# daveredrum/D3Net

Measured on AMD Instinct MI355X. Metric: scenes/sec fwd+bwd (PointGroup+speaker), higher is better.
Workload: dtype bf16

## Files before the change

d3net_amd/_lib.py:

```python
import ctypes as C
import os

_HERE = os.path.dirname(os.path.abspath(__file__))
SO_PATH = os.path.join(_HERE, "lib", "libd3hip.so")

ERRORS = {-1: "D3_ERR_WORKSPACE", -2: "D3_ERR_RANGE (coordinate/batch outside key range)",
          -3: "D3_ERR_ARG", -4: "D3_ERR_OVERFLOW"}


class D3Error(RuntimeError):
    pass


_lib = None
vp, i32, i64, f32, sz = C.c_void_p, C.c_int, C.c_longlong, C.c_float, C.c_size_t
f64 = C.c_double
pi = C.POINTER(C.c_int)

SIGNATURES = {
    "d3_version": (i32, []),
    "d3_arch": (C.c_char_p, []),
    "d3_sec_mean": (i32, [vp, vp, vp, i32, i32, vp]),
    "d3_sec_min": (i32, [vp, vp, vp, i32, i32, vp]),
    "d3_sec_max": (i32, [vp, vp, vp, i32, i32, vp]),
# ... 84 lines not shown
    "d3_point_heads_ws_bytes": (sz, []),
    "d3_point_heads_fwd": (i32, [vp, i64, i32, i32, vp, vp, vp, vp, vp, vp, vp, vp, f32, f32, i32, vp, vp, vp, vp, vp, vp, vp, vp, vp,
                                 vp, sz, vp]),
    "d3_score_loss": (i32, [vp, vp, i32, i32, f32, f32, vp, vp, vp, vp]),
    "d3_query_locals_mask": (i32, [vp, vp, i32, i32, i32, vp]),
    "d3_caption_select_target": (i32, [vp, vp, vp, i32, i32, i32, i32, vp, vp, vp, vp]),
    "d3_caption_inputs_fwd": (i32, [vp, vp, vp, vp, vp, i32, i32, i32, i32, i32, vp, vp, vp, vp, vp]),
    "d3_caption_inputs_bwd": (i32, [vp, vp, vp, vp, i32, i32, i32, i32, i32, vp, vp, vp]),
    "d3_masked_xe_ws_bytes": (sz, [i32, i32]),
    "d3_masked_xe": (i32, [vp, vp, i64, vp, i32, i32, i32, vp, vp, vp, sz, vp]),
    "d3_orientation_loss": (i32, [vp, i64, i64, vp, vp, vp, vp, vp, vp, i32, i32, i32, i32, i32, vp, i32, vp, vp, vp]),
    "d3_offset_loss_ws_bytes": (sz, []),
    "d3_offset_loss": (i32, [vp, vp, vp, i32, vp, i64, vp, vp, vp, i32, vp, sz, vp]),
    "d3_scatter_add_rows": (i32, [vp, vp, vp, i64, i32, vp]),
    "d3_gather_rows": (i32, [vp, vp, vp, i64, i32, vp]),
    "d3_cross_entropy_ws_bytes": (sz, []),
    "d3_cross_entropy": (i32, [vp, vp, vp, vp, i32, i32, i32, vp, sz, vp]),
    "d3_attn_fwd": (i32, [vp, vp, vp, vp, vp, vp, vp, i32, i32, i32, i32, i32, i32, i32, vp]),
    "d3_attn_bwd": (i32, [vp, vp, vp, vp, vp, vp, vp, vp, vp, i32, i32, i32, i32, i32, i32, vp]),
    "d3_hgemm": (i32, [vp, i32, vp]),
    "d3_colsum_ws_bytes": (sz, [i32]),
    "d3_colsum": (i32, [vp, i64, i32, i32, vp, i32, vp, sz, vp]),
    "d3_topdown_ws_bytes": (sz, [i32, i32, i32, i32, i32, i32]),
    "d3_topdown_bwd_ws_bytes": (sz, [i32, i32, i32, i32, i32, i32, i32]),
    "d3_topdown_xe_forward": (i32, [vp, vp]),
    "d3_topdown_xe_backward": (i32, [vp, vp, vp]),
    "d3_topdown_xe_backward_ex": (i32, [vp, vp, vp, vp]),
    "d3_topdown_step_ws_bytes": (sz, [i32, i32, i32, i32, i32]),
    "d3_topdown_feat_proj": (i32, [vp, vp, vp, i32, i32, i32, vp]),
    "d3_topdown_step": (i32, [vp, vp, vp, i32, vp, vp, vp, vp, vp, vp, vp, sz, vp]),
    "d3_beam_select": (i32, [vp, vp, i32, i32, i32, i32, i32, i32, i32, i32, vp, vp, vp, vp, vp, vp, vp, vp, vp, vp, i32, vp]),
    "d3_greedy_select": (i32, [vp, i32, i32, vp, vp, vp]),
    "d3_topdown_greedy": (i32, [vp, vp, i32, vp, vp, vp, vp, vp, vp, vp, sz, vp, i32, vp, vp, vp]),
    "d3_topdown_beam": (i32, [vp, vp, i32, vp, vp, vp, vp, vp, sz, vp, i32, i32, vp, vp, vp, vp, vp, vp, vp]),
    "d3_topdown_beam_greedy": (i32, [vp, vp, i32, vp, vp, vp, vp, vp, sz, vp, i32, i32, vp, vp, vp, vp, vp, vp, i32, vp, vp, vp]),
    "d3_gru_seq_ws_bytes": (sz, [i32, i32, i32, i32]),
    "d3_gru_seq_bwd_ws_bytes": (sz, [i32, i32, i32, i32]),
    "d3_gru_seq_forward": (i32, [vp, vp, vp, vp, vp, vp, i32, i32, i32, i32, vp, vp, vp, sz, vp]),
    "d3_gru_seq_backward": (i32, [vp, vp, vp, vp, i32, i32, i32, i32, vp, vp, vp, vp, vp, vp, vp, vp, vp, sz, vp]),
    "d3_nms3d_samecls": (i32, [vp, vp, vp, i32, i32, f64, i32, vp, vp]),
    "d3_instance_cross_iou": (i32, [vp, vp, i64, i32, i32, vp, vp, vp, vp]),
    "d3_nms_matrix": (i32, [vp, vp, vp, i32, f32, vp, vp, vp, vp]),
    "d3_seg_eval_max_inst": (i32, []),
    "d3_seg_eval_ws_bytes": (sz, [i32, i32]),
    "d3_seg_eval": (i32, [vp, vp, vp, vp, i32, i32, i32, i32, vp, i32, vp, vp, i32, i64, C.c_ulonglong, vp, vp, vp, vp, vp, vp, sz, vp]),
    "d3_scene_limits": (i32, [pi, pi, pi]),
# ... 124 lines not shown
```

d3net_amd/csrc/topdown.hip:

```cpp
#include "common.h"
#include "prof.h"
#include <string.h>

typedef float f32x4 __attribute__((ext_vector_type(4)));
#ifndef GRU_U
#define GRU_U 2
#endif

int hg_launch(const d3_gemm_prob *probs, int nprobs, hipStream_t s);
size_t hg_colsum_ws_bytes(int njobs, int cmax);
int hg_colsum_multi(const float *const *x, const long long *ld, const int *R, const int *C, float *const *out, const int *accum, int n,
                    void *ws, size_t ws_bytes, hipStream_t s);

struct GruArgs {
    const float *x; long long ldx; int I;
    const float *h; long long ldh;
    const float *Wih, *Whh, *bih, *bhh;
    float *hout; long long ldo;
    float *r, *z, *n, *ghn;
    int N, H;
    const float *gi_pre; long long ldgi;
    const int *lens; int t_step;
    float *hid_out; long long ldhid;
    const float *xb; long long ldxb; int Ib; long long ldw;
// ... 235 lines not shown
                                        float *__restrict__ dgi, long long lddgi, float *__restrict__ dgh, float *__restrict__ dhp,
                                        int N, int H, const int *__restrict__ lens, int t_step) {
    const int e = blockIdx.x * blockDim.x + threadIdx.x;
    if (e >= N * H) return;
    const int row = e / H, c = e - row * H;
    float dh = 0.f;
    if (d0) dh += d0[(long long)row * ld0 + c];
    if (d1 && !(lens && t_step >= lens[row])) dh += d1[(long long)row * ld1 + c];
    if (d2) dh += d2[(long long)row * ld2 + c];
    const float rr = r[e], zz = z[e], nv = n[e];
    const float dn = dh * (1.f - zz), dz = dh * (hp[(long long)row * ldh + c] - nv);
    const float dnp = dn * (1.f - nv * nv);
    const float drp = dnp * ghn[e] * rr * (1.f - rr);
    const float dzp = dz * zz * (1.f - zz);
    const long long o = (long long)row * 3 * H + c, oi = (long long)row * lddgi + c;
    dgi[oi] = drp; dgi[oi + H] = dzp; dgi[oi + 2 * H] = dnp;
    dgh[o] = drp; dgh[o + H] = dzp; dgh[o + 2 * H] = dnp * rr;
    dhp[e] = dh * zz;
}

#define TD_PREP_T 1024
__global__ __launch_bounds__(TD_PREP_T) void td_attn_prep_kernel(const float *__restrict__ mask, const float *__restrict__ obj,
                                                                 int *__restrict__ act, int *__restrict__ nact, float *__restrict__ msum,
                                                                 int K, int F, int obj_div) {
    extern __shared__ float sm[];
    const int n = blockIdx.x, t = threadIdx.x, lane = t & 63;
    const long long ns = n / obj_div;
    if (t < 64) {
        int base = 0;
        for (int k0 = 0; k0 < K; k0 += 64) {
            const int k = k0 + lane;
            const bool on = k < K && mask[(long long)n * K + k] != 0.f;
            const unsigned long long bal = __ballot(on);
            if (on) act[(long long)n * K + base + __popcll(bal & ((1ull << lane) - 1ull))] = k;
            base += __popcll(bal);
        }
        if (lane == 0) nact[n] = base;
    }
    const int nsl = TD_PREP_T / F, sl = t / F, c = t - sl * F;
    if (sl < nsl) {
        const int per = (K + nsl - 1) / nsl, k0 = sl * per, k1 = min(K, k0 + per);
        float s = 0.f;
        int k = k0;
        for (; k + 4 <= k1; k += 4) {
            float v[4], m[4];
#pragma unroll
            for (int q = 0; q < 4; q++) { v[q] = obj[(ns * K + k + q) * F + c]; m[q] = mask[(long long)n * K + k + q]; }
#pragma unroll
            for (int q = 0; q < 4; q++) s += (m[q] == 0.f) ? v[q] : 0.f;
        }
        for (; k < k1; k++)
            if (mask[(long long)n * K + k] == 0.f) s += obj[(ns * K + k) * F + c];
        sm[sl * F + c] = s;
    }
    __syncthreads();
    if (t < F) {
        float s = sm[t];
        for (int q = 1; q < nsl; q++) s += sm[q * F + t];
        msum[(long long)n * F + t] = s;
    }
}

#ifndef TD_ATT_T
#define TD_ATT_T 1024
#endif
static inline size_t td_attn_bwd_rsum_floats(int H) { const int CT = H < TD_ATT_T ? H : TD_ATT_T, RS = TD_ATT_T / CT; return RS > 1 ? (size_t)RS * 2 * H : 0; }
template <int NTH>
__global__ __launch_bounds__(NTH) void td_attn_fwd_kernel(const float *__restrict__ fp, const float *__restrict__ q, long long ldq,
                                                          const float *__restrict__ watt, const float *__restrict__ obj,
                                                          const int *__restrict__ act, const int *__restrict__ nact,
                                                          const float *__restrict__ msum, float *__restrict__ a_out,
                                                          float *__restrict__ att, long long ldatt, float *__restrict__ attn_out,
                                                          int t_step, int S, int K, int H, int F, int obj_div) {
    extern __shared__ float sm[];
    float *qs = sm, *ws = qs + H, *sc = ws + H, *ak = sc + K, *part = ak + K;
    __shared__ float am_s;
    const int n = blockIdx.x, t = threadIdx.x, lane = t & 63, wave = t >> 6;
    const long long ns = n / obj_div;
    const int na = nact[n], nm = K - na;
    const int *al = act + (long long)n * K;
    for (int c = t; c < H; c += NTH) { qs[c] = q[(long long)n * ldq + c]; ws[c] = watt[c]; }
    __syncthreads();
    for (int j = wave; j < na; j += NTH / 64) {
        const float *row = fp + (ns * K + al[j]) * H;
        float s = 0.f;
        for (int c = lane * 4; c < H; c += 256) {
            const f32x4 v = *(const f32x4 *)(row + c);
#pragma unroll
            for (int u = 0; u < 4; u++) s += ws[c + u] * tanhf(v[u] + qs[c + u]);
        }
        for (int o = 32; o > 0; o >>= 1) s += __shfl_xor(s, o);
        if (lane == 0) sc[j] = s;
    }
    __syncthreads();
    if (wave == 0) {
        float mx = nm > 0 ? 0.f : -3.0e38f;
        for (int j = lane; j < na; j += 64) mx = fmaxf(mx, sc[j]);
        for (int o = 32; o > 0; o >>= 1) mx = fmaxf(mx, __shfl_xor(mx, o));
        float sum = 0.f;
        for (int j = lane; j < na; j += 64) { const float e = expf(sc[j] - mx); sc[j] = e; sum += e; }
        for (int o = 32; o > 0; o >>= 1) sum += __shfl_xor(sum, o);
        const float e0 = expf(-mx);
        sum += (float)nm * e0;
        const float inv = 1.f / sum;
        for (int j = lane; j < na; j += 64) sc[j] *= inv;
        if (lane == 0) am_s = e0 * inv;
    }
    __syncthreads();
    const float am = am_s;
    for (int k = t; k < K; k += NTH) ak[k] = am;
    __syncthreads();
    for (int j = t; j < na; j += NTH) ak[al[j]] = sc[j];
    __syncthreads();
    for (int k = t; k < K; k += NTH) {
        a_out[(long long)n * K + k] = ak[k];
        if (attn_out) attn_out[((long long)n * K + k) * S + t_step] = ak[k];
    }
    const int half = t / F, c = t - half * F;
    if (half < 2) {
        const int j0 = half * ((na + 1) / 2), j1 = min(na, j0 + (na + 1) / 2);
        float s = 0.f;
        for (int j = j0; j < j1; j++) s += sc[j] * obj[(ns * K + al[j]) * F + c];
        part[half * F + c] = s;
    }
    __syncthreads();
    if (t < F) att[(long long)n * ldatt + t] = am * msum[(long long)n * F + t] + (part[t] + part[F + t]);
}

template <int NTH>
__global__ __launch_bounds__(NTH) void td_attn_bwd_kernel(const float *__restrict__ datt, long long lddatt, const float *__restrict__ a_in,
                                                          const float *__restrict__ att, long long ldatt, const float *__restrict__ fp,
                                                          const float *__restrict__ q, long long ldq, const float *__restrict__ watt,
                                                          const float *__restrict__ obj, const int *__restrict__ act,
                                                          const int *__restrict__ nact, float *__restrict__ dq, long long lddq,
                                                          float *__restrict__ dfp, float *__restrict__ dwpart, float *__restrict__ dattS,
                                                          int K, int H, int F) {
    extern __shared__ float sm[];
    float *dat = sm, *dss = dat + F, *red = dss + K, *rsum = red + 4;
    const int n = blockIdx.x, t = threadIdx.x, lane = t & 63, wave = t >> 6;
    const int na = nact[n];
    const int *al = act + (long long)n * K;
    float pd = 0.f;
    for (int c = t; c < F; c += NTH) {
        const float v = datt[(long long)n * lddatt + c];
        dat[c] = v; dattS[(long long)n * F + c] = v;
        pd += v * att[(long long)n * ldatt + c];
    }
    for (int o = 32; o > 0; o >>= 1) pd += __shfl_xor(pd, o);
    if (lane == 0 && wave < 4) red[wave] = pd;
    __syncthreads();
    const float dot = (red[0] + red[1]) + (red[2] + red[3]);
    for (int j = wave; j < na; j += NTH / 64) {
        const int k = al[j];
        float s = 0.f;
        for (int c = lane; c < F; c += 64) s += dat[c] * obj[((long long)n * K + k) * F + c];
        for (int o = 32; o > 0; o >>= 1) s += __shfl_xor(s, o);
        if (lane == 0) dss[j] = a_in[(long long)n * K + k] * (s - dot);
    }
    __syncthreads();
    const int CT = H < NTH ? H : NTH, RS = NTH / CT, rs = t / CT;
    for (int c = t - rs * CT; c < H && rs < RS; c += CT) {
        const float qc = q[(long long)n * ldq + c], wc = watt[c];
        float dqa = 0.f, dwa = 0.f;
        for (int j0 = rs * 4; j0 < na; j0 += 4 * RS) {
            float fv[4], dv[4];
            long long o[4];
#pragma unroll
            for (int u = 0; u < 4; u++) {
                const int j = j0 + u < na ? j0 + u : j0;
                o[u] = ((long long)n * K + al[j]) * H + c;
                fv[u] = fp[o[u]]; dv[u] = dfp[o[u]];
            }
#pragma unroll
            for (int u = 0; u < 4; u++) {
                if (j0 + u < na) {
                    const float ds = dss[j0 + u];
                    const float th = tanhf(fv[u] + qc);
                    const float dp = ds * wc * (1.f - th * th);
                    dfp[o[u]] = dv[u] + dp;
                    dqa += dp; dwa += ds * th;
                }
            }
        }
        if (rs == 0 && RS == 1) { dq[(long long)n * lddq + c] = dqa; dwpart[(long long)n * H + c] = dwa; }
        else if (rs > 0) { rsum[((rs - 1) * 2) * H + c] = dqa; rsum[((rs - 1) * 2 + 1) * H + c] = dwa; }
        else { rsum[(RS - 1) * 2 * H + c] = dqa; rsum[(RS - 1) * 2 * H + H + c] = dwa; }
    }
    if (RS > 1) {
        __syncthreads();
        for (int c = t; c < H; c += NTH) {
            float dqa = rsum[(RS - 1) * 2 * H + c], dwa = rsum[(RS - 1) * 2 * H + H + c];
            for (int r = 1; r < RS; r++) { dqa += rsum[((r - 1) * 2) * H + c]; dwa += rsum[((r - 1) * 2 + 1) * H + c]; }
            dq[(long long)n * lddq + c] = dqa;
            dwpart[(long long)n * H + c] = dwa;
        }
    }
}

__global__ __launch_bounds__(256) void td_dobj_kernel(const float *__restrict__ a, const float *__restrict__ dattS, float *__restrict__ dobj,
                                                      int S, int N, int K, int F, int SC) {
    extern __shared__ float sm[];
    float *aS = sm, *dS = aS + (size_t)SC * K;
    const int n = blockIdx.x, t = threadIdx.x;
    const int c = t % F, kb = t / F, kst = 256 / F;
    for (int s0 = 0; s0 < S; s0 += SC) {
        const int sc = min(SC, S - s0);
        __syncthreads();
        for (int e = t; e < sc * K; e += 256) { const int tt = e / K, k = e - tt * K; aS[e] = a[((long long)(s0 + tt) * N + n) * K + k]; }
        for (int e = t; e < sc * F; e += 256) { const int tt = e / F, cc = e - tt * F; dS[e] = dattS[((long long)(s0 + tt) * N + n) * F + cc]; }
        __syncthreads();
        const int kper = (K + gridDim.y - 1) / gridDim.y, k0 = blockIdx.y * kper, k1 = min(K, k0 + kper);
        for (int k = k0 + kb; k < k1; k += kst) {
            float v = 0.f;
            for (int tt = 0; tt < sc; tt++) v += aS[tt * K + k] * dS[tt * F + c];
            float *o = dobj + ((long long)n * K + k) * F + c;
            *o = s0 == 0 ? v : *o + v;
        }
    }
// ... 20 lines not shown
    const long long e = (long long)blockIdx.x * blockDim.x + threadIdx.x;
    if (e < n && c0[e] <= 0.f) d[e] = 0.f;
}
__global__ void td_sum_time_kernel(const float *__restrict__ x, float *__restrict__ out, int S, int N, int C) {
    const int e = blockIdx.x * blockDim.x + threadIdx.x;
    if (e >= N * C) return;
    float s = 0.f;
    for (int tt = 0; tt < S; tt++) s += x[(long long)tt * N * C + e];
    out[e] = s;
}

static d3_gemm_seg td_seg(const float *A, long long lda, const float *B, long long ldb, int K, const int *ia = nullptr, int akm = 0, int bkm = 0) {
    d3_gemm_seg s;
    s.A = A; s.ia = ia; s.lda = lda; s.a_kmajor = akm; s.B = B; s.ldb = ldb; s.b_kmajor = bkm; s.K = K;
    return s;
}
static d3_gemm_prob td_prob(int M, int N, float *C, long long ldc) {
    d3_gemm_prob p;
    memset(&p, 0, sizeof(p));
    p.M = M; p.N = N; p.C = C; p.ldc = ldc;
    return p;
}

struct TdLayout {
    size_t widx, nidx, bidx, act, nact, msum, fp, TD, x1, x2, H1, H2, g1, g2, q, a, att, c0, gi1, Wa, Wb, bc2, total;
};
static TdLayout td_layout(int N, int K, int S, int H, int E, int F) {
    TdLayout L;
    size_t o = 0;
    const size_t R = (size_t)S * N;
    auto take = [&](size_t bytes) { size_t at = o; o += d3_align(bytes); return at; };
    L.widx = take(R * 4); L.nidx = take(R * 4); L.bidx = take(R * 4);
    L.act = take((size_t)N * K * 4); L.nact = take((size_t)N * 4); L.msum = take((size_t)N * F * 4);
    L.fp = take((size_t)N * K * H * 4);
    L.TD = take(R * E * 4); L.x1 = take(R * E * 4); L.x2 = take(R * E * 4);
    L.H1 = take((R + N) * H * 4); L.H2 = take((R + N) * H * 4);
    L.g1 = take(4 * R * H * 4); L.g2 = take(4 * R * H * 4);
    L.q = take(R * H * 4); L.a = take(R * K * 4); L.att = take(R * F * 4); L.c0 = take(R * H * 4);
    L.gi1 = take(R * 3 * H * 4); L.Wa = take((size_t)3 * H * (F + H) * 4); L.Wb = take((size_t)3 * H * H * 4); L.bc2 = take((size_t)3 * H * 4);
    L.total = o;
    return L;
}

extern "C" size_t d3_topdown_ws_bytes(int N, int K, int S, int H, int E, int F) {
    return td_layout(N, K, S, H, E, F).total;
}

static int td_check(const d3_topdown_args *a) {
    if (!a || a->N < 1 || a->K < 1 || a->S < 1 || a->V < 1 || a->S > a->Tw) return D3_ERR_ARG;
    if ((a->H & 15) || (a->E & 3) || (a->F & 3) || a->F > 128 || (256 % a->F) || a->K > 1024) return D3_ERR_ARG;
    if (a->ws_bytes < td_layout(a->N, a->K, a->S, a->H, a->E, a->F).total) return D3_ERR_WORKSPACE;
    return 0;
}

extern "C" int d3_topdown_xe_forward(const d3_topdown_args *a, void *stream) {
    D3_CLEAR();
    int rc = td_check(a);
    if (rc) return rc;
    hipStream_t s = d3_stream(stream);
    const int N = a->N, K = a->K, S = a->S, V = a->V, H = a->H, E = a->E, F = a->F, R = S * N;
    const TdLayout L = td_layout(N, K, S, H, E, F);
    char *ws = (char *)a->ws;
    int *widx = (int *)(ws + L.widx), *nidx = (int *)(ws + L.nidx), *bidx = (int *)(ws + L.bidx);
    float *fp = (float *)(ws + L.fp), *TD = (float *)(ws + L.TD), *x1 = (float *)(ws + L.x1), *x2 = (float *)(ws + L.x2);
    float *H1 = (float *)(ws + L.H1), *H2 = (float *)(ws + L.H2), *g1 = (float *)(ws + L.g1), *g2 = (float *)(ws + L.g2);
    float *q = (float *)(ws + L.q), *av = (float *)(ws + L.a), *att = (float *)(ws + L.att), *c0 = (float *)(ws + L.c0);
    int *act = (int *)(ws + L.act), *nact = (int *)(ws + L.nact);
    float *msum = (float *)(ws + L.msum);
    const long long ldtd = H + F + E;
    const long long ldlang = F + H;
    td_rows_kernel<<<(R + 255) / 256, 256, 0, s>>>(a->word_ids, a->Tw, N, S, V, widx, nidx, bidx);
    td_attn_prep_kernel<<<N, TD_PREP_T, (size_t)(TD_PREP_T / F) * F * 4, s>>>(a->mask, a->obj, act, nact, msum, K, F, 1);
    D3_CHECK(hipMemsetAsync(H1, 0, (size_t)N * H * 4, s));
    D3_CHECK(hipMemsetAsync(H2, 0, (size_t)N * H * 4, s));
    {
        d3_gemm_prob p[2];
        p[0] = td_prob(N * K, H, fp, H);
        p[0].nseg = 1; p[0].seg[0] = td_seg(a->obj, F, a->W_feat, F, F);
        p[1] = td_prob(R, E, TD, E);
        p[1].nseg = 2;
        p[1].seg[0] = td_seg(a->emb, E, a->W_td, ldtd, E, widx);
        p[1].seg[1] = td_seg(a->target, F, a->W_td + E + H, ldtd, F, nidx);
        p[1].bias = a->b_td;
        if ((rc = hg_launch(&p[0], 1, s))) return rc;
        if ((rc = hg_launch(&p[1], 1, s))) return rc;
    }
    float *gi1 = (float *)(ws + L.gi1), *Wa = (float *)(ws + L.Wa), *Wb = (float *)(ws + L.Wb), *bc2 = (float *)(ws + L.bc2);
    {
        d3_gemm_prob p[4];
        p[0] = td_prob(3 * H, F + H, Wa, F + H);
        p[0].nseg = 1; p[0].seg[0] = td_seg(a->Wih2, E, a->W_lang, ldlang, E, nullptr, 0, 1);
        p[1] = td_prob(3 * H, H, Wb, H);
        p[1].nseg = 1; p[1].seg[0] = td_seg(a->Wih1, E, a->W_td + E, ldtd, E, nullptr, 0, 1);
        p[2] = td_prob(3 * H, 1, bc2, 1);
        p[2].nseg = 1; p[2].seg[0] = td_seg(a->Wih2, E, a->b_lang, E, E);
        p[2].add = a->bih2; p[2].ldadd = 1;
        p[3] = td_prob(R, 3 * H, gi1, 3 * H);
        p[3].nseg = 1; p[3].seg[0] = td_seg(TD, E, a->Wih1, E, E);
        p[3].bias = a->bih1;
        if ((rc = hg_launch(p, 3, s))) return rc;
        if ((rc = hg_launch(&p[3], 1, s))) return rc;
    }
    const size_t RH = (size_t)R * H;
    for (int t = 0; t < S; t++) {
        const size_t rN = (size_t)t * N;
        float *h1p = H1 + rN * H, *h1n = H1 + (rN + N) * H, *h2p = H2 + rN * H, *h2n = H2 + (rN + N) * H;
        {
            GruArgs g{h2p, H, H, h1p, H, Wb, a->Whh1, nullptr, a->bhh1, h1n, H,
                      g1 + rN * H, g1 + RH + rN * H, g1 + 2 * RH + rN * H, g1 + 3 * RH + rN * H, N, H, gi1 + rN * 3 * H, 3 * H, nullptr, 0, nullptr, 0,
                      nullptr, 0, 0, H};
            if ((rc = td_gru_fwd(g, s))) return rc;
        }
        {
            d3_gemm_prob p = td_prob(N, H, q + rN * H, H);
            p.nseg = 1; p.seg[0] = td_seg(h1n, H, a->W_hidd, H, H);
            if ((rc = hg_launch(&p, 1, s))) return rc;
        }
        td_attn_fwd_kernel<TD_ATT_T><<<N, TD_ATT_T, (size_t)(2 * H + 2 * K + 2 * F) * 4, s>>>(fp, q + rN * H, H, a->w_att, a->obj, act, nact, msum, av + rN * K,
                                                                             att + rN * F, F, a->attn, t, S, K, H, F, 1);
        {
            GruArgs g{att + rN * F, F, F, h2p, H, Wa, a->Whh2, bc2, a->bhh2, h2n, H,
                      g2 + rN * H, g2 + RH + rN * H, g2 + 2 * RH + rN * H, g2 + 3 * RH + rN * H, N, H, nullptr, 0, nullptr, 0, nullptr, 0,
                      h1n, H, H, F + H};
            if ((rc = td_gru_fwd(g, s))) return rc;
        }
    }
    {
        d3_gemm_prob p[2];
        p[0] = td_prob(R, E, x1, E);
        p[0].nseg = 1; p[0].seg[0] = td_seg(H2, H, a->W_td + E, ldtd, H);
        p[0].add = TD; p[0].ldadd = E;
        p[1] = td_prob(R, E, x2, E);
        p[1].nseg = 2;
        p[1].seg[0] = td_seg(att, F, a->W_lang, ldlang, F);
        p[1].seg[1] = td_seg(H1 + (size_t)N * H, H, a->W_lang + F, ldlang, H);
        p[1].bias = a->b_lang;
        if ((rc = hg_launch(p, 2, s))) return rc;
    }
    {
        d3_gemm_prob p = td_prob(R, H, c0, H);
        p.nseg = 1; p.seg[0] = td_seg(H2 + (size_t)N * H, H, a->Wc0, H, H);
        p.bias = a->bc0; p.relu = 1;
// ... 75 lines not shown
    if ((rc = fork(0))) return rc;
    {
        const long long tot = (long long)R * V;
        td_gather_rows_kernel<<<(int)((tot + 255) / 256), 256, 0, sp>>>(gd->dlogits, bidx, dlog, R, V);
        d3_gemm_prob p[3];
        p[0] = td_prob(V, H, gd->dWc2, H);
        p[0].nseg = 1; p[0].seg[0] = td_seg(dlog, V, c0, H, R, nullptr, 1, 1);
        p[1] = td_prob(H, H, gd->dWc0, H);
        p[1].nseg = 1; p[1].seg[0] = td_seg(dc0, H, H2 + (size_t)N * H, H, R, nullptr, 1, 1);
        p[2] = td_prob(R, H, dH2, H);
        p[2].nseg = 1; p[2].seg[0] = td_seg(dc0, H, a->Wc0, H, H, nullptr, 0, 1);
        if ((rc = hg_launch(&p[2], 1, s))) return rc;
        if ((rc = hg_launch(&p[0], 1, sp))) return rc;
        if ((rc = hg_launch(&p[1], 1, sp))) return rc;
        const float *cx[2] = {dlog, dc0}; const long long cl[2] = {V, H}; const int cr[2] = {R, R}, cc[2] = {V, H};
        float *co[2] = {gd->dbc2, gd->dbc0};
        if ((rc = hg_colsum_multi(cx, cl, cr, cc, co, nullptr, 2, bw + B.cs, B.cs_bytes, sp))) return rc;
    }
    D3_CHECK(hipMemsetAsync(dh1c, 0, (size_t)N * H * 4, s));
    D3_CHECK(hipMemsetAsync(dh2c, 0, (size_t)N * H * 4, s));
    D3_CHECK(hipMemsetAsync(dfp, 0, (size_t)N * K * H * 4, s));
    const int nh = (N * H + 255) / 256;
    const bool fuse = d3_tune(D3T_TD_FUSE_GATES) != 0;
    auto gates_epi = [&](d3_gemm_prob &p, const float *d0, long long ld0, const float *d1, long long ld1, const float *g, size_t rN,
                         const float *hp, float *dgi, float *dgh, float *dhp) {
        p.gru = 1; p.gru_H = H;
        p.g_d0 = d0; p.g_ld0 = ld0; p.g_d1 = d1; p.g_ld1 = ld1;
        p.g_r = g + rN * H; p.g_z = g + RH + rN * H; p.g_n = g + 2 * RH + rN * H; p.g_ghn = g + 3 * RH + rN * H;
        p.g_hp = hp; p.g_ldh = H;
        p.g_dgi = dgi; p.g_lddgi = 3 * H; p.g_dgh = dgh; p.g_dhp = dhp;
    };
    for (int t = S - 1; t >= 0; t--) {
        const size_t rN = (size_t)t * N;
        float *h1p = H1 + rN * H, *h2p = H2 + rN * H;
        if (!fuse || t == S - 1)
            td_gru_bwd_gates_kernel<<<nh, 256, 0, s>>>(dH2 + rN * H, H, dh2c, H, nullptr, 0, g2 + rN * H, g2 + RH + rN * H, g2 + 2 * RH + rN * H,
                                                       g2 + 3 * RH + rN * H, h2p, H, dgi2 + rN * 3 * H, 3 * H, dgh2 + rN * 3 * H, dh2c, N, H, nullptr, 0);
        {
            d3_gemm_prob p[3];
            p[0] = td_prob(N, H, dh2c, H);
            p[0].nseg = 1; p[0].seg[0] = td_seg(dgh2 + rN * 3 * H, 3 * H, a->Whh2, H, 3 * H, nullptr, 0, 1); p[0].accum = 1;
            p[1] = td_prob(N, F + H, tmpL, F + H);
            p[1].nseg = 1; p[1].seg[0] = td_seg(dgi2 + rN * 3 * H, 3 * H, Wa, F + H, 3 * H, nullptr, 0, 1);
            p[2] = td_prob(N, E, dx2 + rN * E, E);
            p[2].nseg = 1; p[2].seg[0] = td_seg(dgi2 + rN * 3 * H, 3 * H, a->Wih2, E, 3 * H, nullptr, 0, 1);
            if ((rc = hg_launch(p, 3, s))) return rc;
        }
        td_attn_bwd_kernel<TD_ATT_T><<<N, TD_ATT_T, (size_t)(F + K + 4 + td_attn_bwd_rsum_floats(H)) * 4, s>>>(tmpL, F + H, av + rN * K, att + rN * F, F, fp, q + rN * H, H, a->w_att,
                                                                 a->obj, act, nact, dq + rN * H, H, dfp, dwp + rN * H, dattS + rN * F, K, H, F);
        {
            d3_gemm_prob p = td_prob(N, H, dh1q, H);
            p.nseg = 1; p.seg[0] = td_seg(dq + rN * H, H, a->W_hidd, H, H, nullptr, 0, 1);
            if (fuse) gates_epi(p, dh1c, H, tmpL + F, F + H, g1, rN, h1p, dgi1 + rN * 3 * H, dgh1 + rN * 3 * H, dh1c);
            if ((rc = hg_launch(&p, 1, s))) return rc;
        }
        if (!fuse)
            td_gru_bwd_gates_kernel<<<nh, 256, 0, s>>>(dh1c, H, tmpL + F, F + H, dh1q, H, g1 + rN * H, g1 + RH + rN * H, g1 + 2 * RH + rN * H,
                                                       g1 + 3 * RH + rN * H, h1p, H, dgi1 + rN * 3 * H, 3 * H, dgh1 + rN * 3 * H, dh1c, N, H, nullptr, 0);
        {
            d3_gemm_prob p[3];
            p[0] = td_prob(N, H, dh1c, H);
            p[0].nseg = 1; p[0].seg[0] = td_seg(dgh1 + rN * 3 * H, 3 * H, a->Whh1, H, 3 * H, nullptr, 0, 1); p[0].accum = 1;
            p[1] = td_prob(N, H, dh2c, H);
            p[1].nseg = 1; p[1].seg[0] = td_seg(dgi1 + rN * 3 * H, 3 * H, Wb, H, 3 * H, nullptr, 0, 1); p[1].accum = 1;
            if (fuse && t > 0) {
                const size_t rP = (size_t)(t - 1) * N;
                gates_epi(p[1], dH2 + rP * H, H, nullptr, 0, g2, rP, H2 + rP * H, dgi2 + rP * 3 * H, dgh2 + rP * 3 * H, dh2c);
            }
            p[2] = td_prob(N, E, dx1 + rN * E, E);
            p[2].nseg = 1; p[2].seg[0] = td_seg(dgi1 + rN * 3 * H, 3 * H, a->Wih1, E, 3 * H, nullptr, 0, 1);
            if ((rc = hg_launch(p, 3, s))) return rc;
        }
    }
// ... 29 lines not shown
        p[2] = td_prob(H, H, gd->dW_hidd, H); p[2].nseg = 1; p[2].seg[0] = td_seg(dq, H, H1 + (size_t)N * H, H, R, nullptr, 1, 1);
        p[3] = td_prob(E, H, gd->dW_td + E, ldtd); p[3].nseg = 1; p[3].seg[0] = td_seg(dx1, E, H2, H, R, nullptr, 1, 1);
        if ((rc = hg_launch(p, 4, sp))) return rc;
    }
    {
        d3_gemm_prob p[2];
        p[0] = td_prob(E, F, gd->dW_td + E + H, ldtd); p[0].nseg = 1; p[0].seg[0] = td_seg(dx1s, E, a->target, F, N, nullptr, 1, 1);
        p[1] = td_prob(H, F, gd->dW_feat, F); p[1].nseg = 1; p[1].seg[0] = td_seg(dfp, H, a->obj, F, N * K, nullptr, 1, 1);
        if ((rc = hg_launch(p, 2, sp))) return rc;
    }
    {
        float *embg = dlog;
        const long long tot = (long long)R * E;
        td_gather_rows_kernel<<<(int)((tot + 255) / 256), 256, 0, sp>>>(a->emb, widx, embg, R, E);
        d3_gemm_prob p = td_prob(E, E, gd->dW_td, ldtd);
        p.nseg = 1; p.seg[0] = td_seg(dx1, E, embg, E, R, nullptr, 1, 1);
        if ((rc = hg_launch(&p, 1, sp))) return rc;
    }
    D3_LAUNCH_CHECK();
    return 0;
}

extern "C" size_t d3_topdown_step_ws_bytes(int N, int K, int H, int E, int F) {
    return 2 * d3_align((size_t)N * 4) + 2 * d3_align((size_t)N * E * 4) + 2 * d3_align((size_t)N * H * 4) + 2 * d3_align((size_t)N * F * 4) +
           d3_align((size_t)N * K * 4) + 256;
}

extern "C" int d3_topdown_feat_proj(const float *obj, const float *W_feat, float *fp, int rows, int H, int F, void *stream) {
    D3_CLEAR();
    d3_gemm_prob p = td_prob(rows, H, fp, H);
    p.nseg = 1; p.seg[0] = td_seg(obj, F, W_feat, F, F);
    return hg_launch(&p, 1, d3_stream(stream));
}

__global__ void td_word_idx_kernel(const long long *__restrict__ word, int *__restrict__ widx, int N, int V) {
    const int n = blockIdx.x * blockDim.x + threadIdx.x;
    if (n < N) { const long long w = word[n]; widx[n] = (int)(w < 0 ? 0 : w >= V ? V - 1 : w); }
}

extern "C" int d3_topdown_step(const d3_topdown_args *a, const long long *word, const float *fp, int obj_div, const float *h1_in,
                               const float *h2_in, float *h1_out, float *h2_out, float *logits, float *attn, void *ws_, size_t ws_bytes,
                               void *stream) {
    D3_CLEAR();
    if (!a || a->N < 1 || (a->H & 15) || (a->E & 3) || (a->F & 3) || a->F > 128 || obj_div < 1) return D3_ERR_ARG;
    const int N = a->N, K = a->K, V = a->V, H = a->H, E = a->E, F = a->F;
    if (ws_bytes < d3_topdown_step_ws_bytes(N, K, H, E, F)) return D3_ERR_WORKSPACE;
    hipStream_t s = d3_stream(stream);
    D3Carver cv(ws_, ws_bytes);
    int *widx = cv.take<int>(N);
    float *x1 = cv.take<float>((size_t)N * E), *x2 = cv.take<float>((size_t)N * E), *q = cv.take<float>((size_t)N * H);
    float *c0 = cv.take<float>((size_t)N * H), *att = cv.take<float>((size_t)N * F), *msum = cv.take<float>((size_t)N * F);
    int *act = cv.take<int>((size_t)N * K), *nact = cv.take<int>(N);
    const long long ldtd = H + F + E, ldlang = F + H;
    int rc;
    if (256 % F) return D3_ERR_ARG;
    td_word_idx_kernel<<<(N + 255) / 256, 256, 0, s>>>(word, widx, N, V);
    td_attn_prep_kernel<<<N, TD_PREP_T, (size_t)(TD_PREP_T / F) * F * 4, s>>>(a->mask, a->obj, act, nact, msum, K, F, obj_div);
    {
        d3_gemm_prob p = td_prob(N, E, x1, E);
        p.nseg = 3;
        p.seg[0] = td_seg(a->emb, E, a->W_td, ldtd, E, widx);
        p.seg[1] = td_seg(h2_in, H, a->W_td + E, ldtd, H);
        p.seg[2] = td_seg(a->target, F, a->W_td + E + H, ldtd, F);
        p.bias = a->b_td;
        if ((rc = hg_launch(&p, 1, s))) return rc;
    }
    {
        GruArgs g{x1, E, E, h1_in, H, a->Wih1, a->Whh1, a->bih1, a->bhh1, h1_out, H, nullptr, nullptr, nullptr, nullptr, N, H, nullptr, 0, nullptr, 0, nullptr, 0};
        if ((rc = td_gru_fwd(g, s))) return rc;
    }
    {
        d3_gemm_prob p = td_prob(N, H, q, H);
        p.nseg = 1; p.seg[0] = td_seg(h1_out, H, a->W_hidd, H, H);
        if ((rc = hg_launch(&p, 1, s))) return rc;
    }
    td_attn_fwd_kernel<TD_ATT_T><<<N, TD_ATT_T, (size_t)(2 * H + 2 * K + 2 * F) * 4, s>>>(fp, q, H, a->w_att, a->obj, act, nact, msum, attn, att, F, nullptr, 0, 1, K, H,
                                                                         F, obj_div);
    {
        d3_gemm_prob p = td_prob(N, E, x2, E);
        p.nseg = 2;
        p.seg[0] = td_seg(att, F, a->W_lang, ldlang, F);
        p.seg[1] = td_seg(h1_out, H, a->W_lang + F, ldlang, H);
        p.bias = a->b_lang;
        if ((rc = hg_launch(&p, 1, s))) return rc;
    }
    {
        GruArgs g{x2, E, E, h2_in, H, a->Wih2, a->Whh2, a->bih2, a->bhh2, h2_out, H, nullptr, nullptr, nullptr, nullptr, N, H, nullptr, 0, nullptr, 0, nullptr, 0};
        if ((rc = td_gru_fwd(g, s))) return rc;
    }
    {
        d3_gemm_prob p = td_prob(N, H, c0, H);
        p.nseg = 1; p.seg[0] = td_seg(h2_out, H, a->Wc0, H, H);
        p.bias = a->bc0; p.relu = 1;
        if ((rc = hg_launch(&p, 1, s))) return rc;
        d3_gemm_prob p2 = td_prob(N, V, logits, V);
        p2.nseg = 1; p2.seg[0] = td_seg(c0, H, a->Wc2, H, H);
        p2.bias = a->bc2;
        if ((rc = hg_launch(&p2, 1, s))) return rc;
    }
    D3_LAUNCH_CHECK();
// ... 360 lines not shown
```

include/d3hip.h:

```cpp
#ifndef D3HIP_H
#define D3HIP_H
#include <stddef.h>
#include <stdint.h>

#ifdef __cplusplus
extern "C" {
#endif

#define D3_ERR_WORKSPACE (-1)
#define D3_ERR_RANGE     (-2)
#define D3_ERR_ARG       (-3)
#define D3_ERR_OVERFLOW  (-4)

int d3_version(void);
const char *d3_arch(void);

int d3_sec_mean(const float *inp, const int *offsets, float *out, int nProposal, int C, void *stream);
int d3_sec_min(const float *inp, const int *offsets, float *out, int nProposal, int C, void *stream);
int d3_sec_max(const float *inp, const int *offsets, float *out, int nProposal, int C, void *stream);
int d3_cluster_select(const float *locs, const float *pt_offsets, const int64_t *semantic_preds, const int *batch_idxs,
                      const int64_t *object_idxs, int n, int *batch_out, float *coords_out, float *shifted_out, int *semantic_out,
                      void *stream);
int d3_cluster_select2(const float *locs, const float *pt_offsets, const int64_t *semantic_preds, const int *batch_idxs,
                       const int64_t *object_idxs, int n, int batch_size, int *batch_out, float *coords_out, float *shifted_out,
// ... 246 lines not shown
    const long long *word_ids;
    const float *emb;
    const float *target;
    const float *obj;
    const float *mask;
    const float *W_td, *b_td;
    const float *Wih1, *Whh1, *bih1, *bhh1;
    const float *W_feat, *W_hidd, *w_att;
    const float *W_lang, *b_lang;
    const float *Wih2, *Whh2, *bih2, *bhh2;
    const float *Wc0, *bc0, *Wc2, *bc2;
    float *logits;
    float *attn;
    void *ws; size_t ws_bytes;
} d3_topdown_args;
typedef struct {
    const float *dlogits;
    float *dW_td, *db_td, *dWih1, *dWhh1, *dbih1, *dbhh1, *dW_feat, *dW_hidd, *dw_att, *dW_lang, *db_lang;
    float *dWih2, *dWhh2, *dbih2, *dbhh2, *dWc0, *dbc0, *dWc2, *dbc2;
    float *dobj, *dtarget;
    void *ws; size_t ws_bytes;
} d3_topdown_grads;
size_t d3_topdown_ws_bytes(int N, int K, int S, int H, int E, int F);
size_t d3_topdown_bwd_ws_bytes(int N, int K, int S, int V, int H, int E, int F);
int d3_topdown_xe_forward(const d3_topdown_args *a, void *stream);
int d3_topdown_xe_backward(const d3_topdown_args *a, const d3_topdown_grads *g, void *stream);
int d3_topdown_xe_backward_ex(const d3_topdown_args *a, const d3_topdown_grads *g, void *stream, void *side);
size_t d3_topdown_step_ws_bytes(int N, int K, int H, int E, int F);
int d3_topdown_feat_proj(const float *obj, const float *W_feat, float *fp, int rows, int H, int F, void *stream);
int d3_topdown_step(const d3_topdown_args *a, const long long *word, const float *fp, int obj_div, const float *h1_in,
                    const float *h2_in, float *h1_out, float *h2_out, float *logits, float *attn, void *ws, size_t ws_bytes,
                    void *stream);

int d3_beam_select(const float *logits, const float *sums_in, int N, int live, int b, int V, int eos, int last, int t, int Tmax,
                   const long long *seq_prev, long long *seq_out, long long *tok_out, float *snap_out, unsigned char *ended_out,
                   float *sums_out, const float *h1_in, const float *h2_in, float *h1_out, float *h2_out, int H, void *stream);
int d3_greedy_select(const float *logits, int N, int V, long long *word, float *lp, void *stream);
int d3_topdown_greedy(const d3_topdown_args *a, const float *fp, int obj_div, float *h1_a, float *h2_a, float *h1_b, float *h2_b,
                      float *logits, float *attn, void *ws, size_t ws_bytes, const long long *first_word, int max_len,
                      long long *words, float *lps, void *stream);
int d3_topdown_beam(const d3_topdown_args *a, const float *fp, int b, float *const *h1, float *const *h2, float *logits, float *attn,
                    void *ws, size_t ws_bytes, const long long *first_word, int eos, int max_len, long long *allseq, float *snap_all,
                    unsigned char *ended_all, float *sums0, float *sums1, long long *tok, void *stream);
int d3_topdown_beam_greedy(const d3_topdown_args *a, const float *fp, int b, float *const *h1, float *const *h2, float *logits,
                           float *attn, void *ws, size_t ws_bytes, const long long *first_word, int eos, int max_len,
                           long long *allseq, float *snap_all, unsigned char *ended_all, float *sums0, float *sums1, long long *tok,
// ... 107 lines not shown
```

Before: 248.8.

## Fold W_hidd projection into attention kernels with split-grid score reduction

For small batch (N<=128) the separate GEMM computing q = h1·W_hidd is folded into the attention forward kernel, and the attention score computation is split across a 2D grid whose partial sums are combined by the last block through an atomic counter. In backward the dq·W_hidd^T product and the GRU gate epilogue are fused into the attention backward kernel, which is split over column groups. H1/H2 zeroing and counter reset move into the prep kernel, replacing two memsets. The aim is fewer launches and more parallelism per sequence step, at the cost of redundant per-block work, extra workspace, and last-block synchronization complexity.

```diff
diff --git a/d3net_amd/_lib.py b/d3net_amd/_lib.py
--- a/d3net_amd/_lib.py
+++ b/d3net_amd/_lib.py
@@ -130,6 +130,7 @@
     "d3_colsum_ws_bytes": (sz, [i32]),
     "d3_colsum": (i32, [vp, i64, i32, i32, vp, i32, vp, sz, vp]),
     "d3_topdown_ws_bytes": (sz, [i32, i32, i32, i32, i32, i32]),
+    "d3_topdown_ws_offset": (sz, [i32, i32, i32, i32, i32, i32, i32]),
     "d3_topdown_bwd_ws_bytes": (sz, [i32, i32, i32, i32, i32, i32, i32]),
     "d3_topdown_xe_forward": (i32, [vp, vp]),
     "d3_topdown_xe_backward": (i32, [vp, vp, vp]),
diff --git a/d3net_amd/csrc/topdown.hip b/d3net_amd/csrc/topdown.hip
--- a/d3net_amd/csrc/topdown.hip
+++ b/d3net_amd/csrc/topdown.hip
@@ -281,10 +281,14 @@
 #define TD_PREP_T 1024
 __global__ __launch_bounds__(TD_PREP_T) void td_attn_prep_kernel(const float *__restrict__ mask, const float *__restrict__ obj,
                                                                  int *__restrict__ act, int *__restrict__ nact, float *__restrict__ msum,
-                                                                 int K, int F, int obj_div) {
+                                                                 int K, int F, int obj_div, int *__restrict__ cnt,
+                                                                 float *__restrict__ z1, float *__restrict__ z2, int H) {
     extern __shared__ float sm[];
     const int n = blockIdx.x, t = threadIdx.x, lane = t & 63;
     const long long ns = n / obj_div;
+    if (t == 0) cnt[n] = 0;
+    if (z1)
+        for (int c = t; c < H; c += TD_PREP_T) { z1[(long long)n * H + c] = 0.f; z2[(long long)n * H + c] = 0.f; }
     if (t < 64) {
         int base = 0;
         for (int k0 = 0; k0 < K; k0 += 64) {
@@ -323,33 +327,92 @@
 #ifndef TD_ATT_T
 #define TD_ATT_T 1024
 #endif
+#define TD_FOLD_MAX_N 128
+static inline int td_attn_split(int N) { return N <= 32 ? 8 : N <= 64 ? 4 : N <= TD_FOLD_MAX_N ? 2 : 1; }
 static inline size_t td_attn_bwd_rsum_floats(int H) { const int CT = H < TD_ATT_T ? H : TD_ATT_T, RS = TD_ATT_T / CT; return RS > 1 ? (size_t)RS * 2 * H : 0; }
 template <int NTH>
-__global__ __launch_bounds__(NTH) void td_attn_fwd_kernel(const float *__restrict__ fp, const float *__restrict__ q, long long ldq,
+__global__ __launch_bounds__(NTH) void td_attn_fwd_kernel(const float *__restrict__ fp, float *__restrict__ q, long long ldq,
+                                                          const float *__restrict__ h1, long long ldh1, const float *__restrict__ Whid,
+                                                          float *spart, int *cnt,
                                                           const float *__restrict__ watt, const float *__restrict__ obj,
                                                           const int *__restrict__ act, const int *__restrict__ nact,
                                                           const float *__restrict__ msum, float *__restrict__ a_out,
                                                           float *__restrict__ att, long long ldatt, float *__restrict__ attn_out,
                                                           int t_step, int S, int K, int H, int F, int obj_div) {
     extern __shared__ float sm[];
-    float *qs = sm, *ws = qs + H, *sc = ws + H, *ak = sc + K, *part = ak + K;
+    float *qs = sm, *ws = qs + H, *hs = ws + H, *sc = hs + H, *ak = sc + K, *part = ak + K;
     __shared__ float am_s;
+    __shared__ int last_s;
     const int n = blockIdx.x, t = threadIdx.x, lane = t & 63, wave = t >> 6;
+    const int G = gridDim.y, g = blockIdx.y, LG = 64 / G;
     const long long ns = n / obj_div;
     const int na = nact[n], nm = K - na;
     const int *al = act + (long long)n * K;
-    for (int c = t; c < H; c += NTH) { qs[c] = q[(long long)n * ldq + c]; ws[c] = watt[c]; }
-    __syncthreads();
-    for (int j = wave; j < na; j += NTH / 64) {
-        const float *row = fp + (ns * K + al[j]) * H;
-        float s = 0.f;
-        for (int c = lane * 4; c < H; c += 256) {
-            const f32x4 v = *(const f32x4 *)(row + c);
-#pragma unroll
-            for (int u = 0; u < 4; u++) s += ws[c + u] * tanhf(v[u] + qs[c + u]);
-        }
-        for (int o = 32; o > 0; o >>= 1) s += __shfl_xor(s, o);
-        if (lane == 0) sc[j] = s;
+    if (Whid) {
+        for (int c = t; c < H; c += NTH) { hs[c] = h1[(long long)n * ldh1 + c]; ws[c] = watt[c]; }
+        __syncthreads();
+        const int CW = 4 * LG, nown = CW * ((H + 255) >> 8);
+        for (int m0 = wave * 4; m0 < nown; m0 += (NTH / 64) * 4) {
+            const int p = m0 / CW, c0 = 256 * p + CW * g + (m0 - p * CW);
+            if (c0 >= H) continue;
+            const float *w0 = Whid + (long long)c0 * H;
+            float s[4] = {0.f, 0.f, 0.f, 0.f};
+#pragma unroll 2
+            for (int k = lane * 4; k < H; k += 256) {
+                const f32x4 hv = *(const f32x4 *)(hs + k);
+                f32x4 wv[4];
+#pragma unroll
+                for (int u = 0; u < 4; u++) wv[u] = *(const f32x4 *)(w0 + (long long)u * H + k);
+#pragma unroll
+                for (int u = 0; u < 4; u++)
+#pragma unroll
+                    for (int e = 0; e < 4; e++) s[u] += wv[u][e] * hv[e];
+            }
+#pragma unroll
+            for (int u = 0; u < 4; u++)
+                for (int o = 32; o > 0; o >>= 1) s[u] += __shfl_xor(s[u], o);
+            if (lane < 4) { const float v = lane == 0 ? s[0] : lane == 1 ? s[1] : lane == 2 ? s[2] : s[3]; qs[c0 + lane] = v; q[(long long)n * ldq + c0 + lane] = v; }
+        }
+    } else {
+        for (int c = t; c < H; c += NTH) { qs[c] = q[(long long)n * ldq + c]; ws[c] = watt[c]; }
+    }
+    __syncthreads();
+    if (G == 1) {
+        for (int j = wave; j < na; j += NTH / 64) {
+            const float *row = fp + (ns * K + al[j]) * H;
+            float s = 0.f;
+            for (int c = lane * 4; c < H; c += 256) {
+                const f32x4 v = *(const f32x4 *)(row + c);
+#pragma unroll
+                for (int u = 0; u < 4; u++) s += ws[c + u] * tanhf(v[u] + qs[c + u]);
+            }
+            for (int o = 32; o > 0; o >>= 1) s += __shfl_xor(s, o);
+            if (lane == 0) sc[j] = s;
+        }
+    } else {
+        float *sp = spart + (long long)n * K * 64;
+        for (int e = t; e < na * LG; e += NTH) {
+            const int j = e / LG, ln = g * LG + (e - j * LG);
+            const float *row = fp + (ns * K + al[j]) * H;
+            float s = 0.f;
+            for (int c = ln * 4; c < H; c += 256) {
+                const f32x4 v = *(const f32x4 *)(row + c);
+#pragma unroll
+                for (int u = 0; u < 4; u++) s += ws[c + u] * tanhf(v[u] + qs[c + u]);
+            }
+            __hip_atomic_store(sp + j * 64 + ln, s, __ATOMIC_RELAXED, __HIP_MEMORY_SCOPE_AGENT);
+        }
+        asm volatile("s_waitcnt vmcnt(0)" ::: "memory");
+        __syncthreads();
+        if (t == 0) last_s = __hip_atomic_fetch_add(cnt + n, 1, __ATOMIC_RELAXED, __HIP_MEMORY_SCOPE_AGENT) == G - 1;
+        __syncthreads();
+        if (!last_s) return;
+        if (t == 0) cnt[n] = 0;
+        for (int j = wave; j < na; j += NTH / 64) {
+            float s = __hip_atomic_load(sp + j * 64 + lane, __ATOMIC_RELAXED, __HIP_MEMORY_SCOPE_AGENT);
+            for (int o = 32; o > 0; o >>= 1) s += __shfl_xor(s, o);
+            if (lane == 0) sc[j] = s;
+        }
     }
     __syncthreads();
     if (wave == 0) {
@@ -386,6 +449,12 @@
     if (t < F) att[(long long)n * ldatt + t] = am * msum[(long long)n * F + t] + (part[t] + part[F + t]);
 }
 
+struct TdGateArgs {
+    const float *d0, *d1; long long ld1;
+    const float *g; long long gs;
+    const float *hp;
+    float *dgi, *dgh, *dhp;
+};
 template <int NTH>
 __global__ __launch_bounds__(NTH) void td_attn_bwd_kernel(const float *__restrict__ datt, long long lddatt, const float *__restrict__ a_in,
                                                           const float *__restrict__ att, long long ldatt, const float *__restrict__ fp,
@@ -393,16 +462,21 @@
                                                           const float *__restrict__ obj, const int *__restrict__ act,
                                                           const int *__restrict__ nact, float *__restrict__ dq, long long lddq,
                                                           float *__restrict__ dfp, float *__restrict__ dwpart, float *__restrict__ dattS,
-                                                          int K, int H, int F) {
+                                                          int K, int H, int F, const float *__restrict__ Whid, float *__restrict__ dh1q,
+                                                          const TdGateArgs gt) {
     extern __shared__ float sm[];
     float *dat = sm, *dss = dat + F, *red = dss + K, *rsum = red + 4;
     const int n = blockIdx.x, t = threadIdx.x, lane = t & 63, wave = t >> 6;
+    const int G = gridDim.y, g = blockIdx.y, CW = H / G, own0 = g * CW;
+    const int CT = H < NTH ? H : NTH, RS = NTH / CT, rs = t / CT;
+    float *dqs = rsum + (RS > 1 ? RS * 2 * H : 0), *psum = dqs + H;
     const int na = nact[n];
     const int *al = act + (long long)n * K;
     float pd = 0.f;
     for (int c = t; c < F; c += NTH) {
         const float v = datt[(long long)n * lddatt + c];
-        dat[c] = v; dattS[(long long)n * F + c] = v;
+        dat[c] = v;
+        if (g == 0) dattS[(long long)n * F + c] = v;
         pd += v * att[(long long)n * ldatt + c];
     }
     for (int o = 32; o > 0; o >>= 1) pd += __shfl_xor(pd, o);
@@ -417,8 +491,8 @@
         if (lane == 0) dss[j] = a_in[(long long)n * K + k] * (s - dot);
     }
     __syncthreads();
-    const int CT = H < NTH ? H : NTH, RS = NTH / CT, rs = t / CT;
     for (int c = t - rs * CT; c < H && rs < RS; c += CT) {
+        const bool own = c >= own0 && c < own0 + CW;
         const float qc = q[(long long)n * ldq + c], wc = watt[c];
         float dqa = 0.f, dwa = 0.f;
         for (int j0 = rs * 4; j0 < na; j0 += 4 * RS) {
@@ -428,7 +502,7 @@
             for (int u = 0; u < 4; u++) {
                 const int j = j0 + u < na ? j0 + u : j0;
                 o[u] = ((long long)n * K + al[j]) * H + c;
-                fv[u] = fp[o[u]]; dv[u] = dfp[o[u]];
+                fv[u] = fp[o[u]]; dv[u] = own ? dfp[o[u]] : 0.f;
             }
 #pragma unroll
             for (int u = 0; u < 4; u++) {
@@ -436,12 +510,15 @@
                     const float ds = dss[j0 + u];
                     const float th = tanhf(fv[u] + qc);
                     const float dp = ds * wc * (1.f - th * th);
-                    dfp[o[u]] = dv[u] + dp;
+                    if (own) dfp[o[u]] = dv[u] + dp;
                     dqa += dp; dwa += ds * th;
                 }
             }
         }
-        if (rs == 0 && RS == 1) { dq[(long long)n * lddq + c] = dqa; dwpart[(long long)n * H + c] = dwa; }
+        if (rs == 0 && RS == 1) {
+            if (own) { dq[(long long)n * lddq + c] = dqa; dwpart[(long long)n * H + c] = dwa; }
+            if (Whid) dqs[c] = dqa;
+        }
         else if (rs > 0) { rsum[((rs - 1) * 2) * H + c] = dqa; rsum[((rs - 1) * 2 + 1) * H + c] = dwa; }
         else { rsum[(RS - 1) * 2 * H + c] = dqa; rsum[(RS - 1) * 2 * H + H + c] = dwa; }
     }
@@ -450,9 +527,44 @@
         for (int c = t; c < H; c += NTH) {
             float dqa = rsum[(RS - 1) * 2 * H + c], dwa = rsum[(RS - 1) * 2 * H + H + c];
             for (int r = 1; r < RS; r++) { dqa += rsum[((r - 1) * 2) * H + c]; dwa += rsum[((r - 1) * 2 + 1) * H + c]; }
-            dq[(long long)n * lddq + c] = dqa;
-            dwpart[(long long)n * H + c] = dwa;
-        }
+            if (c >= own0 && c < own0 + CW) { dq[(long long)n * lddq + c] = dqa; dwpart[(long long)n * H + c] = dwa; }
+            if (Whid) dqs[c] = dqa;
+        }
+    }
+    if (!Whid) return;
+    __syncthreads();
+    const int CWT = CW < NTH ? CW : NTH, JS = NTH / CWT, js = t / CWT, cl = t - js * CWT;
+    for (int cb = 0; cb < CW; cb += CWT) {
+        float s = 0.f;
+        if (js < JS && cb + cl < CW) {
+            const float *w = Whid + own0 + cb + cl;
+#pragma unroll 8
+            for (int j = js; j < H; j += JS) s += dqs[j] * w[(long long)j * H];
+        }
+        psum[t] = s;
+        __syncthreads();
+        if (t < CWT && cb + t < CW) {
+            float v = psum[t];
+            for (int r = 1; r < JS; r++) v += psum[r * CWT + t];
+            const int c = own0 + cb + t;
+            if (gt.g) {
+                const long long e = (long long)n * H + c;
+                float dh = 0.f;
+                dh += gt.d0[e];
+                dh += gt.d1[(long long)n * gt.ld1 + c];
+                dh += v;
+                const float rr = gt.g[e], zz = gt.g[gt.gs + e], nv = gt.g[2 * gt.gs + e];
+                const float dn = dh * (1.f - zz), dz = dh * (gt.hp[e] - nv);
+                const float dnp = dn * (1.f - nv * nv);
+                const float drp = dnp * gt.g[3 * gt.gs + e] * rr * (1.f - rr);
+                const float dzp = dz * zz * (1.f - zz);
+                const long long og = (long long)n * 3 * H + c;
+                gt.dgi[og] = drp; gt.dgi[og + H] = dzp; gt.dgi[og + 2 * H] = dnp;
+                gt.dgh[og] = drp; gt.dgh[og + H] = dzp; gt.dgh[og + 2 * H] = dnp * rr;
+                gt.dhp[e] = dh * zz;
+            } else dh1q[(long long)n * H + c] = v;
+        }
+        __syncthreads();
     }
 }
 
@@ -519,8 +631,26 @@
     return p;
 }
 
+static int td_attn_fwd(const float *fp, float *q, const float *h1, const float *Whid, float *spart, int *cnt, const float *watt,
+                       const float *obj, const int *act, const int *nact, const float *msum, float *a_out, float *att, float *attn_out,
+                       int t_step, int S, int N, int K, int H, int F, int obj_div, hipStream_t s) {
+    const size_t lds = (size_t)(3 * H + 2 * K + 2 * F) * 4;
+    if (N > TD_FOLD_MAX_N) {
+        d3_gemm_prob p = td_prob(N, H, q, H);
+        p.nseg = 1; p.seg[0] = td_seg(h1, H, Whid, H, H);
+        int rc = hg_launch(&p, 1, s);
+        if (rc) return rc;
+        td_attn_fwd_kernel<TD_ATT_T><<<N, TD_ATT_T, lds, s>>>(fp, q, H, nullptr, 0, nullptr, nullptr, cnt, watt, obj, act, nact, msum, a_out, att, F,
+                                                             attn_out, t_step, S, K, H, F, obj_div);
+        return 0;
+    }
+    td_attn_fwd_kernel<TD_ATT_T><<<dim3(N, td_attn_split(N)), TD_ATT_T, lds, s>>>(fp, q, H, h1, H, Whid, spart, cnt, watt, obj, act, nact, msum, a_out,
+                                                                                 att, F, attn_out, t_step, S, K, H, F, obj_div);
+    return 0;
+}
+
 struct TdLayout {
-    size_t widx, nidx, bidx, act, nact, msum, fp, TD, x1, x2, H1, H2, g1, g2, q, a, att, c0, gi1, Wa, Wb, bc2, total;
+    size_t widx, nidx, bidx, act, nact, msum, fp, TD, x1, x2, H1, H2, g1, g2, q, a, att, c0, gi1, Wa, Wb, bc2, sp, cnt, total;
 };
 static TdLayout td_layout(int N, int K, int S, int H, int E, int F) {
     TdLayout L;
@@ -535,12 +665,17 @@
     L.g1 = take(4 * R * H * 4); L.g2 = take(4 * R * H * 4);
     L.q = take(R * H * 4); L.a = take(R * K * 4); L.att = take(R * F * 4); L.c0 = take(R * H * 4);
     L.gi1 = take(R * 3 * H * 4); L.Wa = take((size_t)3 * H * (F + H) * 4); L.Wb = take((size_t)3 * H * H * 4); L.bc2 = take((size_t)3 * H * 4);
+    L.sp = take(N <= TD_FOLD_MAX_N ? (size_t)N * K * 64 * 4 : 0); L.cnt = take((size_t)N * 4);
     L.total = o;
     return L;
 }
 
 extern "C" size_t d3_topdown_ws_bytes(int N, int K, int S, int H, int E, int F) {
     return td_layout(N, K, S, H, E, F).total;
+}
+extern "C" size_t d3_topdown_ws_offset(int which, int N, int K, int S, int H, int E, int F) {
+    const TdLayout L = td_layout(N, K, S, H, E, F);
+    return which == 0 ? L.H1 : which == 1 ? L.H2 : which == 2 ? L.q : (size_t)-1;
 }
 
 static int td_check(const d3_topdown_args *a) {
@@ -567,9 +702,9 @@
     const long long ldtd = H + F + E;
     const long long ldlang = F + H;
     td_rows_kernel<<<(R + 255) / 256, 256, 0, s>>>(a->word_ids, a->Tw, N, S, V, widx, nidx, bidx);
-    td_attn_prep_kernel<<<N, TD_PREP_T, (size_t)(TD_PREP_T / F) * F * 4, s>>>(a->mask, a->obj, act, nact, msum, K, F, 1);
-    D3_CHECK(hipMemsetAsync(H1, 0, (size_t)N * H * 4, s));
-    D3_CHECK(hipMemsetAsync(H2, 0, (size_t)N * H * 4, s));
+    float *spart = (float *)(ws + L.sp);
+    int *cnt = (int *)(ws + L.cnt);
+    td_attn_prep_kernel<<<N, TD_PREP_T, (size_t)(TD_PREP_T / F) * F * 4, s>>>(a->mask, a->obj, act, nact, msum, K, F, 1, cnt, H1, H2, H);
     {
         d3_gemm_prob p[2];
         p[0] = td_prob(N * K, H, fp, H);
@@ -608,13 +743,8 @@
                       nullptr, 0, 0, H};
             if ((rc = td_gru_fwd(g, s))) return rc;
         }
-        {
-            d3_gemm_prob p = td_prob(N, H, q + rN * H, H);
-            p.nseg = 1; p.seg[0] = td_seg(h1n, H, a->W_hidd, H, H);
-            if ((rc = hg_launch(&p, 1, s))) return rc;
-        }
-        td_attn_fwd_kernel<TD_ATT_T><<<N, TD_ATT_T, (size_t)(2 * H + 2 * K + 2 * F) * 4, s>>>(fp, q + rN * H, H, a->w_att, a->obj, act, nact, msum, av + rN * K,
-                                                                             att + rN * F, F, a->attn, t, S, K, H, F, 1);
+        if ((rc = td_attn_fwd(fp, q + rN * H, h1n, a->W_hidd, spart, cnt, a->w_att, a->obj, act, nact, msum, av + rN * K, att + rN * F, a->attn, t, S,
+                              N, K, H, F, 1, s))) return rc;
         {
             GruArgs g{att + rN * F, F, F, h2p, H, Wa, a->Whh2, bc2, a->bhh2, h2n, H,
                       g2 + rN * H, g2 + RH + rN * H, g2 + 2 * RH + rN * H, g2 + 3 * RH + rN * H, N, H, nullptr, 0, nullptr, 0, nullptr, 0,
@@ -736,6 +866,7 @@
     D3_CHECK(hipMemsetAsync(dfp, 0, (size_t)N * K * H * 4, s));
     const int nh = (N * H + 255) / 256;
     const bool fuse = d3_tune(D3T_TD_FUSE_GATES) != 0;
+    const bool fold = N <= TD_FOLD_MAX_N;
     auto gates_epi = [&](d3_gemm_prob &p, const float *d0, long long ld0, const float *d1, long long ld1, const float *g, size_t rN,
                          const float *hp, float *dgi, float *dgh, float *dhp) {
         p.gru = 1; p.gru_H = H;
@@ -760,9 +891,17 @@
             p[2].nseg = 1; p[2].seg[0] = td_seg(dgi2 + rN * 3 * H, 3 * H, a->Wih2, E, 3 * H, nullptr, 0, 1);
             if ((rc = hg_launch(p, 3, s))) return rc;
         }
-        td_attn_bwd_kernel<TD_ATT_T><<<N, TD_ATT_T, (size_t)(F + K + 4 + td_attn_bwd_rsum_floats(H)) * 4, s>>>(tmpL, F + H, av + rN * K, att + rN * F, F, fp, q + rN * H, H, a->w_att,
-                                                                 a->obj, act, nact, dq + rN * H, H, dfp, dwp + rN * H, dattS + rN * F, K, H, F);
-        {
+        TdGateArgs gt;
+        memset(&gt, 0, sizeof(gt));
+        if (fold && fuse) {
+            gt.d0 = dh1c; gt.d1 = tmpL + F; gt.ld1 = F + H;
+            gt.g = g1 + rN * H; gt.gs = (long long)RH;
+            gt.hp = h1p; gt.dgi = dgi1 + rN * 3 * H; gt.dgh = dgh1 + rN * 3 * H; gt.dhp = dh1c;
+        }
+        td_attn_bwd_kernel<TD_ATT_T><<<dim3(N, fold ? td_attn_split(N) : 1), TD_ATT_T, (size_t)(F + K + 4 + td_attn_bwd_rsum_floats(H) + H + TD_ATT_T) * 4, s>>>(
+            tmpL, F + H, av + rN * K, att + rN * F, F, fp, q + rN * H, H, a->w_att, a->obj, act, nact, dq + rN * H, H, dfp, dwp + rN * H,
+            dattS + rN * F, K, H, F, fold ? a->W_hidd : nullptr, dh1q, gt);
+        if (!fold) {
             d3_gemm_prob p = td_prob(N, H, dh1q, H);
             p.nseg = 1; p.seg[0] = td_seg(dq + rN * H, H, a->W_hidd, H, H, nullptr, 0, 1);
             if (fuse) gates_epi(p, dh1c, H, tmpL + F, F + H, g1, rN, h1p, dgi1 + rN * 3 * H, dgh1 + rN * 3 * H, dh1c);
@@ -838,8 +977,8 @@
 }
 
 extern "C" size_t d3_topdown_step_ws_bytes(int N, int K, int H, int E, int F) {
-    return 2 * d3_align((size_t)N * 4) + 2 * d3_align((size_t)N * E * 4) + 2 * d3_align((size_t)N * H * 4) + 2 * d3_align((size_t)N * F * 4) +
-           d3_align((size_t)N * K * 4) + 256;
+    return 3 * d3_align((size_t)N * 4) + 2 * d3_align((size_t)N * E * 4) + 2 * d3_align((size_t)N * H * 4) + 2 * d3_align((size_t)N * F * 4) +
+           d3_align((size_t)N * K * 4) + d3_align(N <= TD_FOLD_MAX_N ? (size_t)N * K * 64 * 4 : 0) + 256;
 }
 
 extern "C" int d3_topdown_feat_proj(const float *obj, const float *W_feat, float *fp, int rows, int H, int F, void *stream) {
@@ -866,12 +1005,13 @@
     int *widx = cv.take<int>(N);
     float *x1 = cv.take<float>((size_t)N * E), *x2 = cv.take<float>((size_t)N * E), *q = cv.take<float>((size_t)N * H);
     float *c0 = cv.take<float>((size_t)N * H), *att = cv.take<float>((size_t)N * F), *msum = cv.take<float>((size_t)N * F);
-    int *act = cv.take<int>((size_t)N * K), *nact = cv.take<int>(N);
+    int *act = cv.take<int>((size_t)N * K), *nact = cv.take<int>(N), *cnt = cv.take<int>(N);
+    float *spart = cv.take<float>(N <= TD_FOLD_MAX_N ? (size_t)N * K * 64 : 0);
     const long long ldtd = H + F + E, ldlang = F + H;
     int rc;
     if (256 % F) return D3_ERR_ARG;
     td_word_idx_kernel<<<(N + 255) / 256, 256, 0, s>>>(word, widx, N, V);
-    td_attn_prep_kernel<<<N, TD_PREP_T, (size_t)(TD_PREP_T / F) * F * 4, s>>>(a->mask, a->obj, act, nact, msum, K, F, obj_div);
+    td_attn_prep_kernel<<<N, TD_PREP_T, (size_t)(TD_PREP_T / F) * F * 4, s>>>(a->mask, a->obj, act, nact, msum, K, F, obj_div, cnt, nullptr, nullptr, H);
     {
         d3_gemm_prob p = td_prob(N, E, x1, E);
         p.nseg = 3;
@@ -885,13 +1025,8 @@
         GruArgs g{x1, E, E, h1_in, H, a->Wih1, a->Whh1, a->bih1, a->bhh1, h1_out, H, nullptr, nullptr, nullptr, nullptr, N, H, nullptr, 0, nullptr, 0, nullptr, 0};
         if ((rc = td_gru_fwd(g, s))) return rc;
     }
-    {
-        d3_gemm_prob p = td_prob(N, H, q, H);
-        p.nseg = 1; p.seg[0] = td_seg(h1_out, H, a->W_hidd, H, H);
-        if ((rc = hg_launch(&p, 1, s))) return rc;
-    }
-    td_attn_fwd_kernel<TD_ATT_T><<<N, TD_ATT_T, (size_t)(2 * H + 2 * K + 2 * F) * 4, s>>>(fp, q, H, a->w_att, a->obj, act, nact, msum, attn, att, F, nullptr, 0, 1, K, H,
-                                                                         F, obj_div);
+    if ((rc = td_attn_fwd(fp, q, h1_out, a->W_hidd, spart, cnt, a->w_att, a->obj, act, nact, msum, attn, att, nullptr, 0, 1, N, K, H, F, obj_div, s)))
+        return rc;
     {
         d3_gemm_prob p = td_prob(N, E, x2, E);
         p.nseg = 2;
diff --git a/include/d3hip.h b/include/d3hip.h
--- a/include/d3hip.h
+++ b/include/d3hip.h
@@ -292,6 +292,7 @@
     void *ws; size_t ws_bytes;
 } d3_topdown_grads;
 size_t d3_topdown_ws_bytes(int N, int K, int S, int H, int E, int F);
+size_t d3_topdown_ws_offset(int which, int N, int K, int S, int H, int E, int F);
 size_t d3_topdown_bwd_ws_bytes(int N, int K, int S, int V, int H, int E, int F);
 int d3_topdown_xe_forward(const d3_topdown_args *a, void *stream);
 int d3_topdown_xe_backward(const d3_topdown_args *a, const d3_topdown_grads *g, void *stream);
```

After: 225.6. 9.4% lower.
